# laser55/mrcAudioCodec

Measured on AMD Instinct MI355X. Metric: encode Msamples/sec (48 kHz, 2048-pt MDCT), higher is better.
Workload: dtype f64; 1 GPU; configs[1]: mono 48 kHz white noise (sigma 0.1 FS, 16-bit PCM), 2048-pt long blocks, whole encode path, independent-frames mode; hop=1024

## Files before the change

mrcaudiocodec_amd/csrc/mrc_smr_body.hpp:

```cpp
#pragma once
#include "mrc_smr_sweep.hpp"

#include <type_traits>

namespace mrc {
using namespace dev;
namespace {

constexpr int kLinesPerThread = 4;

constexpr int kSmrWavesPerSimd = 4, kSmrWavesPerSimdShort = 6;
constexpr int kFrontPrio = 3, kFarPrio = 0;

template <bool EXACT, class SampleT, int NT, int DIM, int MODE>
__device__ __forceinline__ void smr_body(DevShape S, int nsigArg, const SampleT* __restrict__ chL,
                                         const SampleT* __restrict__ chR, int64_t stride,
                                         const int64_t* __restrict__ offsetsArg, const double* __restrict__ lines,
                                         const int* __restrict__ oscale, double* __restrict__ smr,
                                         double* __restrict__ threshArg, double* __restrict__ bandPeakArg,
                                         const int* __restrict__ msSwitch, SmrLds layArg,
                                         unsigned long long* __restrict__ sens) {
    extern __shared__ double smem[];
    const SmrLds lay = DIM ? smr_layout(DIM, DIM, DIM - 100, nullptr) : layArg;
    __shared__ int waveCnt[NT / kWave];
    __shared__ unsigned long long bandKey[kMaxBands], peakKey[kMaxBands];
    __shared__ unsigned long long slopeKey[2];
    __shared__ unsigned char needBand[kMaxBands];
    const int tid = threadIdx.x;
    const int lane = tid & (kWave - 1), wave = tid >> 6;
    constexpr bool LONG = DIM == 1024;
    const int nsig = MODE == 1 ? 1 : MODE == 2 ? 4 : nsigArg;
    const bool haveSwitch = MODE == 1 ? false : MODE == 2 ? true : msSwitch != nullptr;
    const int64_t* offsets = offsetsArg;
    double* thresh = MODE ? nullptr : threshArg;
    double* bandPeak = bandPeakArg;
    const bool wantPeak = MODE ? true : bandPeakArg != nullptr;
    const int H = DIM ? DIM : S.H, M = DIM ? DIM : S.halfN;
    const int last = DIM ? DIM - 100 : S.peakLast;
    const unsigned slot = xcd_contiguous(blockIdx.x, gridDim.x);
    const int64_t f = slot / nsig;
    const int sig = (int)((slot + f) % nsig);
    const unsigned unit = (unsigned)(f * nsig + sig);
    if (haveSwitch && !thresh) {
        const bool need = lane < S.nBands && ((sig >= 2) == (msSwitch[f * S.nBands + lane] != 0));
        if (!__any(need)) return;
    }
    const int64_t off = offsets ? offsets[f] : f * stride;
    double2* A = (double2*)smem;
    double2* B = A + H;
    double* xi = smem + 4 * H;
    unsigned short* cntArr = reinterpret_cast<unsigned short*>(smem + 2 * H);
    unsigned short* nUpArr = cntArr + (M + 2);
    short* pkBin = reinterpret_cast<short*>(nUpArr + (M + 2));
    double* piHi = reinterpret_cast<double*>(pkBin + ((last / 2 + 5) & ~3));
    double* piLo = piHi + (last / 2 + 2);

#ifdef MRC_PROFILE_PHASES
    __shared__ unsigned long long sPhase_[32];
    if (threadIdx.x < 32) sPhase_[threadIdx.x] = 0ull;
    __syncthreads();
    long long tPhase_ = __builtin_readcyclecounter();
#endif
    __builtin_amdgcn_s_setprio(kFrontPrio);
    if (tid < kMaxBands) bandKey[tid] = 0ull;
    if (tid < 2) slopeKey[tid] = tid ? 0ull : ~0ull;
    if (tid < kMaxBands) peakKey[tid] = 0ull;
    if (tid < kMaxBands)
        needBand[tid] = (!haveSwitch || tid >= S.nBands) ? 1 : (((sig >= 2) == (msSwitch[f * S.nBands + tid] != 0)) ? 1 : 0);
    const double* zbS = smem + lay.zbOff;
    constexpr int TAB = (DIM == 1024 && !EXACT && NT == 256) ? kExpTabLong : kExpTab;
    constexpr int kTabLongOff = 464;
    const double* e2tab = TAB == kExpTab ? smem + 2 * H - kExpTab : smem + 4 * H + kTabLongOff;
    unsigned long long* ratioKey = reinterpret_cast<unsigned long long*>(smem + 2 * H - kExpTab - kMaxBands);
    const double* logTabLds = smem + lay.logOff;
    const double* logTab = logTabLds;
    constexpr int kPre = 4;
    const bool pairAligned = !(off & 1) && !(reinterpret_cast<uintptr_t>(chL) & (2 * sizeof(SampleT) - 1)) &&
                             (!chR || !(reinterpret_cast<uintptr_t>(chR) & (2 * sizeof(SampleT) - 1)));
    MRC_PHASE(16);
    constexpr bool kFftRegs = LONG && NT == 256 && kPre == 4;
    constexpr bool kSplitPairs = kFftRegs;
    [[maybe_unused]] double2 fftIn[4];
    [[maybe_unused]] Tw3 fftW1;
    if constexpr (kFftRegs) fftW1 = fft1024_twiddles(S.fftTw, 1, tid);
    for (int n0 = tid; n0 < H; n0 += NT * kPre) {
        double e[kPre], o[kPre], he[kPre], ho[kPre];
#pragma unroll
        for (int u = 0; u < kPre; ++u) {
            const int n = min(n0 + u * NT, H - 1);
            const double2 eo = load_signal_pair(chL, chR, off + 2 * n, sig, pairAligned);
            e[u] = eo.x;
            o[u] = eo.y;
            he[u] = S.hann[2 * n];
            ho[u] = S.hann[2 * n + 1];
        }
#pragma unroll
        for (int u = 0; u < kPre; ++u) {
            const int n = n0 + u * NT;
            if constexpr (kFftRegs) fftIn[u] = make_double2(e[u] * he[u], o[u] * ho[u]);
            else if (n < H) A[n] = make_double2(e[u] * he[u], o[u] * ho[u]);
        }
    }
    const int scale = oscale[unit];
    const double xiInv = 1.0 / S.xiDen;
    double2 wnPre[kPre];
    double zbPre[kPre], logPre = 0.0, e2Pre = 0.0;
    [[maybe_unused]] double e2Pre64 = 0.0;
#pragma unroll
    for (int u = 0; u < kPre; ++u) {
        if (!kSplitPairs || u < 2) wnPre[u] = S.wN[kSplitPairs ? tid + 1 + u * NT : min(tid + u * NT, last - 1)];
        zbPre[u] = EXACT ? 0.0 : S.zb[min(tid + u * NT, M - 1)];
    }
    if (!EXACT) {
        logPre = kLogTabDev.v[tid & (kLogTabEntries * 4 - 1)];
        e2Pre = TAB == kExpTab ? kExp2Tab[tid & (kExpTab - 1)] : kExp2Tab256[tid & 255];
        if (TAB != kExpTab) e2Pre64 = kExp2Tab[tid & (kExpTab - 1)];
    }
    double2* T;
    if constexpr (kFftRegs) {
        MRC_PHASE(0); MRC_STOP(0);
        T = fft_regs_1024(fftIn, A, B, S.fftTw, fftW1, tid);
    } else if (lay.twOff >= 0) {
        double2* Wq = reinterpret_cast<double2*>(smem + lay.twOff);
        for (int t = tid; t < H / 4; t += NT) Wq[t] = S.wH[t];
        __syncthreads();
        MRC_PHASE(0); MRC_STOP(0);
        if (LONG && NT == 256) T = fft_lds_1024<NT>(A, B, Wq, tid);
        else if (DIM == 128) T = fft_lds_128<NT>(A, B, Wq, tid);
        else
        T = fft_lds_pow2<NT>(A, B, H, S.radH, S.nRadH, TwQuarter{Wq, H / 4 - 1, 31 - __clz(H / 4)}, tid);
    } else {
        __syncthreads();
        MRC_PHASE(0); MRC_STOP(0);
        if (DIM == 576) T = fft_lds_576<NT>(A, B, S.wH, tid);
        else
        T = fft_lds_global<NT>(A, B, H, S.radH, S.nRadH, S.wH, tid);
    }
    MRC_PHASE(1); MRC_STOP(1);
    if constexpr (kSplitPairs) {
        auto intensity = [&](double2 X) {
            return EXACT ? 4. * (X.x * X.x + X.y * X.y) / S.xiDen : (4. * (X.x * X.x + X.y * X.y)) * xiInv;
        };
        auto split = [&](int k, double2 w, bool both) {
            const double2 zk = T[k];
            double2 zc = T[(H - k) & (H - 1)];
            zc.y = -zc.y;
            const double2 ev = make_double2(0.5 * (zk.x + zc.x), 0.5 * (zk.y + zc.y));
            const double2 d = make_double2(zk.x - zc.x, zk.y - zc.y);
            const double2 od = make_double2(0.5 * d.y, -0.5 * d.x);
            const double2 P = cmul(w, od);
            xi[k] = intensity(make_double2(P.x + ev.x, P.y + ev.y));
            if (both) xi[H - k] = intensity(make_double2(ev.x - P.x, ev.y - P.y));
        };
#pragma unroll
        for (int u = 0; u < 2; ++u) {
            const int k = tid + 1 + u * NT;
            split(k, wnPre[u], H - k < last && k != H / 2);
        }
        if (tid == 0) split(0, make_double2(1.0, 0.0), false);
    } else
    for (int k0 = tid; k0 < last; k0 += NT * kPre) {
        double2 wn[kPre];
#pragma unroll
        for (int u = 0; u < kPre; ++u) wn[u] = (k0 == tid) ? wnPre[u] : S.wN[min(k0 + u * NT, last - 1)];
#pragma unroll
        for (int u = 0; u < kPre; ++u) {
            const int k = k0 + u * NT;
            if (k < last) {
                double2 zk = T[k];
                double2 zc = T[(H - k) % H];
                zc.y = -zc.y;
                double2 ev = make_double2(0.5 * (zk.x + zc.x), 0.5 * (zk.y + zc.y));
                double2 d = make_double2(zk.x - zc.x, zk.y - zc.y);
                double2 od = make_double2(0.5 * d.y, -0.5 * d.x);
                double2 X = cmul(wn[u], od);
                X.x += ev.x; X.y += ev.y;
                xi[k] = EXACT ? 4. * (X.x * X.x + X.y * X.y) / S.xiDen
                              : (4. * (X.x * X.x + X.y * X.y)) * xiInv;
            }
        }
    }
    MRC_PHASE(20);
    __syncthreads();
    MRC_PHASE(2); MRC_STOP(2);
    if (!EXACT) {
        {
            double* zw = smem + lay.zbOff;
#pragma unroll
            for (int u = 0; u < kPre; ++u)
                if (tid + u * NT < M) zw[tid + u * NT] = zbPre[u];
            for (int k = tid + kPre * NT; k < M; k += NT) zw[k] = S.zb[k];
        }
        if (tid < kLogTabEntries * 4) smem[lay.logOff + tid] = logPre;
        if (tid < kExpTab) smem[2 * H - kExpTab + tid] = TAB == kExpTab ? e2Pre : e2Pre64;
        if (tid < kMaxBands) ratioKey[tid] = 0ull;
    }

    double* mt = smem;
    const int nCand = last - 2;
    const int per = (nCand + NT - 1) / NT;
    const int p0 = 1 + tid * per;
    const int p1 = min(p0 + per, last - 1);
    constexpr int kPerMax = 4;
    int mine = 0;
    unsigned flags = 0;
    if (per <= kPerMax) {
        double v[kPerMax + 2];
#pragma unroll
        for (int j = 0; j < kPerMax + 2; ++j) v[j] = xi[min(p0 - 1 + j, last - 1)];
#pragma unroll
        for (int j = 0; j < kPerMax; ++j)
            if (p0 + j < p1 && v[j + 1] > v[j] && v[j + 1] > v[j + 2]) flags |= 1u << j;
        mine = __popc(flags);
        if (sens) {
            const double kPeakGuard = 1e-11 * __longlong_as_double((long long)sens[7]);
            int near = 0;
#pragma unroll
            for (int j = 0; j < kPerMax; ++j) {
                const double c = v[j + 1], l = v[j], r = v[j + 2];
                const bool nl = fabs(c - l) <= kPeakGuard * c, nr = fabs(c - r) <= kPeakGuard * c;
                near += (p0 + j < p1 && ((nl && (c > r || nr)) || (nr && (c > l || nl)))) ? 1 : 0;
            }
            if (near) atomicAdd(&sens[3], (unsigned long long)near);
        }
    } else {
        for (int p = p0; p < p1; ++p) mine += (xi[p] > xi[p - 1] && xi[p] > xi[p + 1]) ? 1 : 0;
    }
    const int incl = wave_incl_scan(mine);
    if (lane == kWave - 1) waveCnt[wave] = incl;
    MRC_PHASE(17);
    __syncthreads();
    MRC_PHASE(18);
    int before = incl - mine, nPeaks = 0;
    for (int w = 0; w < NT / kWave; ++w) {
        const int c = waveCnt[w];
        if (w < wave) before += c;
        nPeaks += c;
    }
    if (per <= kPerMax) {
#pragma unroll
        for (int j = 0; j < kPerMax; ++j)
            if ((flags >> j) & 1u) pkBin[before++] = (short)(p0 + j);
    } else {
        for (int p = p0; p < p1; ++p)
            if (xi[p] > xi[p - 1] && xi[p] > xi[p + 1]) pkBin[before++] = (short)p;
    }
    if (!EXACT) {
        unsigned long long* z = reinterpret_cast<unsigned long long*>(cntArr);
        for (int k = tid; k < (M + 2) / 2; k += NT) z[k] = 0ull;
    }
    MRC_PHASE(19);
    __syncthreads();
    MRC_PHASE(3); MRC_STOP(3);
    double slLo = 1e300, slHi = -1e300;
    for (int mi = tid; mi < nPeaks; mi += NT) {
        const int before = mi;
        const int p = pkBin[mi];
        const double x0 = xi[p - 1], x1 = xi[p], x2 = xi[p + 1];
        {
            double s3 = (x0 + x1) + x2;
            MRC_PHASE(21);
            double level = EXACT ? spl_db(s3) : spl_db_tab(s3, logTabLds);
            const double fnum = S.binHz * (((p - 1) * x0 + p * x1) + (p + 1) * x2);
            double fm = EXACT ? fnum / s3 : fnum * recip_nr(s3);
            double q = EXACT ? fm / 7500. : fm * (1. / 7500.);
            const double zm = EXACT ? 13 * atan(0.76 * fm / 1000.) + 3.5 * atan(q * q)
                                    : 13 * atan_pos((0.76 * fm) * 1e-3) + 3.5 * atan_pos(q * q);
            const double lvl15 = level - 15.0;
            const double boost = 0.37 * fmax(level - 40, 0.0);
            double* e = mt + 4 * before;
            if (EXACT) {
                e[1] = zm;
                e[0] = lvl15;
                e[2] = boost;
            } else {
                const double xe = (lvl15 - 96) * 0.1;
                const double eh = xe * kLog2Of10;
                const double I = exp2_dd(eh, fma(xe, kLog2Of10, -eh) + xe * kLog2Of10Lo);
                const double ph = kLowHi * zm;
                const double pl = fma(kLowHi, zm, -ph) + kLowLo * zm;
                const double slope = (((-27 + boost) * 0.1) * kLog2Of10) * (double)TAB;
                slLo = fmin(slLo, slope);
                slHi = fmax(slHi, slope);
                reinterpret_cast<double2*>(e)[0] = make_double2(I, zm);
                reinterpret_cast<double2*>(e)[1] = make_double2(slope, I * exp2_dd(ph, pl));
                const int kNear = min(max((int)(fm * S.linesPerHz), 0), M - 1);
                MRC_PHASE(22);
                int lo = S.loLine[kNear], hi = S.hiLine[kNear];
#ifdef MRC_PROFILE_PHASES
                asm volatile("" : "+v"(lo), "+v"(hi));
#endif
                MRC_PHASE(23);
                {
                    auto zAt = [&](int k) { return zbS[min(max(k, 0), M - 1)]; };
                    const double a0 = zAt(lo - 2), a1 = zAt(lo - 1), a2 = zAt(lo), a3 = zAt(lo + 1);
                    const double b0 = zAt(hi - 2), b1 = zAt(hi - 1), b2 = zAt(hi), b3 = zAt(hi + 1);
                    auto sees = [&](double zv, int k) { return k >= M || (k >= 0 && zv - zm >= -0.5); };
                    auto above = [&](double zv, int k) { return k >= M || (k >= 0 && zv - zm > 0.5); };
                    const bool s0 = sees(a0, lo - 2), s1 = sees(a1, lo - 1), s2 = sees(a2, lo), s3 = sees(a3, lo + 1);
                    const bool u0 = above(b0, hi - 2), u1 = above(b1, hi - 1), u2 = above(b2, hi), u3 = above(b3, hi + 1);
                    const int first = (s1 && !s0) ? lo - 1 : (s2 && !s1) ? lo : (s3 && !s2) ? lo + 1 : -1;
                    const int over = (u1 && !u0) ? hi - 1 : (u2 && !u1) ? hi : (u3 && !u2) ? hi + 1 : -1;
                    if (__any(first < 0 || over < 0)) {
                        while (lo > 0 && zbS[lo - 1] - zm >= -0.5) --lo;
                        while (lo < M && !(zbS[lo] - zm >= -0.5)) ++lo;
                        hi = max(hi, lo);
                        while (hi > 0 && zbS[hi - 1] - zm > 0.5) --hi;
                        while (hi < M && !(zbS[hi] - zm > 0.5)) ++hi;
                    } else {
                        lo = first;
                        hi = over;
                    }
                }
                atomicAdd(reinterpret_cast<unsigned int*>(cntArr) + (lo >> 1), 1u << (16 * (lo & 1)));
                atomicAdd(reinterpret_cast<unsigned int*>(nUpArr) + (hi >> 1), 1u << (16 * (hi & 1)));
                MRC_PHASE(24);
            }
        }
    }
    if (!EXACT) {
        slLo = -wave_max(-slLo);
        slHi = wave_max(slHi);
        if (lane == 0) {
            atomicMin(&slopeKey[0], order_key(slLo));
            atomicMax(&slopeKey[1], order_key(slHi));
        }
    }
    MRC_PHASE(4);
    __syncthreads();
    MRC_PHASE(12); MRC_STOP(4);

    const double* X = lines + (int64_t)unit * M;

    if (EXACT) {
        for (int base = 0; base < M; base += NT * kLinesPerThread) {
            double z[kLinesPerThread], tot[kLinesPerThread];
#pragma unroll
            for (int j = 0; j < kLinesPerThread; ++j) {
                int k = base + tid + j * NT;
                bool ok = k < M;
                z[j] = ok ? S.zb[k] : 0.0;
                tot[j] = ok ? S.quiet[k] : 0.0;
            }
            for (int m = 0; m < nPeaks; ++m) {
                const double lvl = mt[4 * m], zm = mt[4 * m + 1], boost = mt[4 * m + 2];
#pragma unroll
                for (int j = 0; j < kLinesPerThread; ++j) {
                    double dz = z[j] - zm;
                    double adz = fabs(dz);
                    double t = adz - 0.5;
                    double arg = lvl;
                    if (adz > 0.5) arg = lvl + (-27 * t);
                    if (dz > 0.5) arg = arg + boost * t;
                    tot[j] += pow(10.0, (arg - 96) / 10);
                }
            }
#pragma unroll
            for (int j = 0; j < kLinesPerThread; ++j) {
                int k = base + tid + j * NT;
                if (k < M) {
                    double thr = spl_db(tot[j]);
                    if (thresh) thresh[(int64_t)unit * M + k] = thr;
                    double xs = ldexp(X[k], scale);
                    double spl = spl_db(2. * (xs * xs) / (1. / 2.)) - 6. * scale;
                    atomicMax(&bandKey[S.bandOfLine[k]], order_key(spl - thr));
                    if (wantPeak)
                        atomicMax(&peakKey[S.bandOfLine[k]], (unsigned long long)__double_as_longlong(fabs(X[k])));
                }
            }
        }
    } else {
        double* sc = xi;
        if (TAB != kExpTab) smem[4 * H + kTabLongOff + tid] = e2Pre;
        const int waveU = __builtin_amdgcn_readfirstlane(wave);
        const int nChunks = (M + kWave - 1) / kWave;
        const int nWaves = NT / kWave;
        struct LineConst { double z, quiet, lowE, x; int bnd; };
        auto chunk_of = [&](int i) { return i * nWaves + ((i & 1) ? (nWaves - 1 - waveU) : waveU); };
        auto load_consts = [&](int i) {
            const unsigned kc = (unsigned)min(chunk_of(i) * kWave + lane, M - 1);
            const char* lc = reinterpret_cast<const char*>(S.lineC) + kc * (unsigned)sizeof(LineConstants);
            const double2 a = *reinterpret_cast<const double2*>(lc);
            const double lowE = *reinterpret_cast<const double*>(lc + 16);
            const int bnd = *reinterpret_cast<const int*>(lc + 24);
            const double x = *reinterpret_cast<const double*>(reinterpret_cast<const char*>(X) + kc * 8u);
            return LineConst{a.x, a.y, lowE, x, bnd};
        };
        constexpr bool kFirstEarly = LONG && NT == 256;
        [[maybe_unused]] LineConst first{};
        if constexpr (kFirstEarly) first = load_consts(0);
        constexpr bool kNodes = (DIM == 1024 || DIM == 576) && NT == 256;
        constexpr int kNodeMaxMaskers = kNodes ? node_max_maskers(DIM ? DIM : 1024) : 0;
        static_assert(!kNodes || kNodeMaxMaskers >= 128, "slope nodes: too few rows for this block shape");
        [[maybe_unused]] double nodeH = 0.0, nodeS0 = 0.0;
        bool useNodes = false;
        if constexpr (kNodes) {
            const double lo = order_value(slopeKey[0]), hi = order_value(slopeKey[1]);
            nodeH = fmax((hi - lo) * (1.0 / (kNodeR - 1 - 2 * kNodeMargin)), kNodeHMin * TAB);
            nodeS0 = hi + kNodeMargin * nodeH;
            useNodes = nPeaks >= kNodeMinMaskers && nPeaks <= kNodeMaxMaskers && nodeH <= kNodeHMax * TAB;
        }
        double* const nodeQ = reinterpret_cast<double*>(pkBin);
        double* piH = piHi;
        double* piL = piLo;
        if (kNodes && useNodes) { piH = mt + 4 * nPeaks; piL = piH + (nPeaks + 1); }
        constexpr int kSegAny = DIM == 128 ? 1 : DIM == 576 ? 4 : kSmrMaxSeg;
        constexpr int kSegNodes = DIM == 1024 ? 5 : kSegAny;
        static_assert(DIM != 1024 || kWave * kSegNodes > node_max_maskers(1024), "segments of the scans");
        auto scan_sc = [&](auto segC) {
            constexpr int kSeg = decltype(segC)::value;
            double loc[kSeg];
            double run = 0.0;
            const int seg = kWave - 1 - lane;
#pragma unroll
            for (int i = kSeg - 1; i >= 0; --i) {
                const int m = seg * kSeg + i;
                run += (m < nPeaks) ? mt[4 * m + 3] : 0.0;
                loc[i] = run;
            }
            const double incl = wave_incl_scan(run);
            const double higher = dpp_shift_or_zero<0x138, 0xf>(incl);
#pragma unroll
            for (int i = 0; i < kSeg; ++i) {
                const int m = seg * kSeg + i;
                if (m < nPeaks) sc[m] = loc[i] + higher;
            }
            if (lane == 0) sc[nPeaks] = 0.0;
        };
        auto scan_pi = [&](auto segC) {
            constexpr int kSeg = decltype(segC)::value;
            double hi = 0.0, lo = 0.0, locH[kSeg], locL[kSeg];
#pragma unroll
            for (int i = 0; i < kSeg; ++i) {
                const int m = lane * kSeg + i;
                locH[i] = hi; locL[i] = lo;
                dd_add(&hi, &lo, (m < nPeaks) ? mt[4 * m] : 0.0, 0.0);
            }
            double inH = hi, inL = lo;
#define MRC_DD_SCAN_STEP(CTRL, MASK)                                                           \
            dd_add(&inH, &inL, dpp_shift_or_zero<CTRL, MASK>(inH), dpp_shift_or_zero<CTRL, MASK>(inL));
            MRC_DD_SCAN_STEP(0x111, 0xf) MRC_DD_SCAN_STEP(0x112, 0xf) MRC_DD_SCAN_STEP(0x114, 0xf)
            MRC_DD_SCAN_STEP(0x118, 0xf) MRC_DD_SCAN_STEP(0x142, 0xa) MRC_DD_SCAN_STEP(0x143, 0xc)
#undef MRC_DD_SCAN_STEP
            const double exH = dpp_shift_or_zero<0x138, 0xf>(inH), exL = dpp_shift_or_zero<0x138, 0xf>(inL);
#pragma unroll
            for (int i = 0; i < kSeg; ++i) {
                const int m = lane * kSeg + i;
                if (m <= nPeaks) {
                    double h = exH, l = exL;
                    dd_add(&h, &l, locH[i], locL[i]);
                    piH[m] = h; piL[m] = l;
                }
            }
        };
        auto scan_counts = [&](unsigned short* arr) {
            const int per2 = (M + kWave) / kWave;
            const int k0 = lane * per2, k1 = min(k0 + per2, M + 1);
            int sum = 0;
            for (int k = k0; k < k1; ++k) sum += arr[k];
            int run = wave_incl_scan(sum) - sum;
            for (int k = k0; k < k1; ++k) {
                run += arr[k];
                arr[k] = (unsigned short)run;
            }
        };
        [[maybe_unused]] auto scan_counts_1024 = [&](unsigned short* arr) {
            unsigned* w = reinterpret_cast<unsigned*>(arr) + 8 * lane;
            unsigned x[8];
#pragma unroll
            for (int j = 0; j < 8; ++j) x[j] = w[j];
            unsigned carry = 0;
#pragma unroll
            for (int j = 0; j < 8; ++j) {
                unsigned v = x[j] + (x[j] << 16);
                v += carry * 0x10001u;
                x[j] = v;
                carry = v >> 16;
            }
            const unsigned before = (unsigned)(wave_incl_scan((int)carry) - (int)carry) * 0x10001u;
#pragma unroll
            for (int j = 0; j < 8; ++j) w[j] = x[j] + before;
        };
        [[maybe_unused]] auto node_terms = [&]() {
            const double* tab64 = smem + 2 * H - kExpTab;
            const double invH = 1.0 / nodeH;
            const double s0q = nodeS0 * ((double)kExpTab / TAB), hq = nodeH * ((double)kExpTab / TAB);
            if (tid < kNodeCols) nodeQ[tid] = 0.0;
            for (int base = waveU * kWave; base < nPeaks; base += NT) {
                const int m = base + lane;
                const bool valid = m < nPeaks;
                const int mm = min(m, nPeaks - 1);
                const double2 Iz = *reinterpret_cast<const double2*>(mt + 4 * mm);
                const double I = valid ? Iz.x : 0.0, zm = Iz.y, sl = mt[4 * mm + 2];
                const double theta = (nodeS0 - sl) * invH;
                double suf[kNodeR];
                suf[kNodeR - 1] = 1.0;
#pragma unroll
                for (int r = kNodeR - 2; r >= 0; --r) suf[r] = suf[r + 1] * (theta - (r + 1));
                const double F0 = I * exp2_tab64<kExpTab>(-s0q, zm, tab64);
                const double gm = exp2_tab64<kExpTab>(hq, zm, tab64);
                double G[kNodeCols];
                double F = F0, pre = 1.0, lsum = 0.0;
#pragma unroll
                for (int r = 0; r < kNodeR; ++r) {
                    const double lam = (pre * kNodeW.c[r]) * suf[r];
                    G[r] = lam * F;
                    lsum += fabs(lam);
                    F *= gm;
                    pre *= theta - r;
                }
                G[kNodeR] = I * (fabs(pre) * kInvFactorial[kNodeR]);
                G[kNodeR + 1] = lsum * F0;
                const bool store = (lane & 3) == 0 && valid;
                double* rowOut = nodeQ + ((m >> 2) + 1) * kNodeCols;
#pragma unroll
                for (int j = 0; j < kNodeCols; ++j) {
                    double v = G[j];
                    v += dpp_move<0xB1>(v);
                    v += dpp_move<0x4E>(v);
                    if (store) rowOut[j] = v;
                }
            }
        };
        [[maybe_unused]] auto node_scan = [&](int half) {
            static_assert(kNodeCols == 18 && kNodeScanSegs * 9 <= kWave, "columns of the row scan");
            static_assert((node_max_maskers(1024) + kNodeC - 1) / kNodeC <= kNodeScanSegs * kNodeSeg, "rows of the row scan");
            const int nR = (nPeaks + kNodeC - 1) / kNodeC;
            const int L = (nR + kNodeScanSegs - 1) / kNodeScanSegs;
            const int seg = (lane * 57) >> 9;
            const int col = 9 * half + (lane - 9 * seg);
            const bool live = seg < kNodeScanSegs;
            double v[kNodeSeg];
#pragma unroll
            for (int i = 0; i < kNodeSeg; ++i) {
                const int r = 1 + seg * L + i;
                v[i] = (live && i < L && r <= nR) ? nodeQ[r * kNodeCols + col] : 0.0;
            }
#pragma unroll
            for (int i = 1; i < kNodeSeg; ++i) v[i] += v[i - 1];
            const double tot = v[kNodeSeg - 1];
            auto from_below = [&](double x, int d) {
                const int from = 4 * (lane - 9 * d);
                const double y = __hiloint2double(__builtin_amdgcn_ds_bpermute(from, __double2hiint(x)),
                                                  __builtin_amdgcn_ds_bpermute(from, __double2loint(x)));
                return seg >= d ? y : 0.0;
            };
            double off = from_below(tot, 1);
#pragma unroll
            for (int d = 1; d < kNodeScanSegs; d *= 2) off += from_below(off, d);
#pragma unroll
            for (int i = 0; i < kNodeSeg; ++i) {
                const int r = 1 + seg * L + i;
                if (live && i < L && r <= nR) nodeQ[r * kNodeCols + col] = v[i] + off;
            }
        };
        bool scansDone = false;
        if constexpr (kNodes) {
            if (useNodes) {
                MRC_PHASE(13);
                node_terms();
                MRC_PHASE(14);
                using SegN = std::integral_constant<int, kSegNodes>;
                auto counts = [&](unsigned short* arr) {
                    if constexpr (DIM == 1024) scan_counts_1024(arr); else scan_counts(arr);
                };
                if (nPeaks > NT) {
                    if (waveU == 1) scan_pi(SegN{});
                    else if (waveU == 2) { scan_sc(SegN{}); counts(cntArr); }
                    else if (waveU == 3) counts(nUpArr);
                    MRC_PHASE(9);
                    __syncthreads();
                    MRC_PHASE(15);
                    if (waveU == 2 || waveU == 3) node_scan(waveU - 2);
                } else {
                    __syncthreads();
                    MRC_PHASE(15);
                    if (waveU < 2) node_scan(waveU);
                    else if (waveU == 2) scan_pi(SegN{});
                    else { scan_sc(SegN{}); counts(cntArr); counts(nUpArr); }
                    MRC_PHASE(9);
                }
                scansDone = true;
            }
        }
        if (!scansDone) {
            for (int task = waveU; task < 4; task += NT / kWave) {
                using SegA = std::integral_constant<int, kSegAny>;
                if (task == 0) scan_sc(SegA{});
                else if (task == 1) scan_pi(SegA{});
                else if constexpr (DIM == 1024) scan_counts_1024(task == 2 ? cntArr : nUpArr);
                else scan_counts(task == 2 ? cntArr : nUpArr);
            }
        }
        __syncthreads();
        MRC_PHASE(5); MRC_STOP(5);

        auto tail_sum = [&](double tot, int cnt, int from, double lowE) {
            if (cnt > from) {
                const double ah = piH[cnt], al = piL[cnt], bh = piH[from], bl = piL[from];
                const double d1 = ah - bh;
                const double v = d1 - ah;
                const double e = ((ah - (d1 - v)) - (bh + v)) + (al - bl);
                tot += d1 + e;
            }
            return fma(lowE, sc[cnt], tot);
        };
        auto line_a2 = [&](const LineConst& cur) {
            const double xs2 = ldexp(cur.x, scale + 1);
            return xs2 * xs2;
        };
        auto line_plain = [&](double a2, double t) { return thresh != nullptr || !(a2 >= kSplFloorGuard && t >= kSplFloorGuard); };
        auto finish = [&](const LineConst& cur, int k, double t, auto noPlain) {
            const double a2 = line_a2(cur);
            const bool plain = decltype(noPlain)::value ? false : line_plain(a2, t);
            double ex = -1e300, q = 0.0;
            if (plain) {
                double thr;
                ex = excess_plain(t, a2, scale, logTab, &thr);
                if (thresh && k < M) thresh[(int64_t)unit * M + k] = thr;
            } else {
                q = line_ratio(a2, t);
            }
            const int bnd = cur.bnd;
            if (__all(bnd == __builtin_amdgcn_readfirstlane(bnd))) {
                const bool rowHead = (lane & 15) == 0;
                const double qBest = row_max(q);
                if (rowHead) atomicMax(&ratioKey[bnd], (unsigned long long)__double_as_longlong(qBest));
                if (__any(plain)) {
                    const double best = row_max(ex);
                    if (rowHead) atomicMax(&bandKey[bnd], order_key(best));
                }
                if (wantPeak) {
                    const double pk = row_max(fabs(cur.x));
                    if (rowHead) atomicMax(&peakKey[bnd], (unsigned long long)__double_as_longlong(pk));
                }
            } else {
                atomicMax(&ratioKey[bnd], (unsigned long long)__double_as_longlong(q));
                if (plain) atomicMax(&bandKey[bnd], order_key(ex));
                if (wantPeak) atomicMax(&peakKey[bnd], (unsigned long long)__double_as_longlong(fabs(cur.x)));
            }
        };
        __builtin_amdgcn_s_setprio(0);
        const double slMid = 0.5 * (order_value(slopeKey[0]) + order_value(slopeKey[1]));
        const double spreadHalf = 0.5 * (order_value(slopeKey[1]) - order_value(slopeKey[0])) * (0.6931471805599453094 / TAB);
        if (kNodes && useNodes) {
            if constexpr (kNodes) {
            MRC_NODE_COUNT(0);
            const double xr = (nodeH * kNodeR) / (-nodeS0);
            double ps = xr * xr;
            ps *= ps; ps *= ps; ps *= ps;
            const double psiStar = ps * kExpMinus16;
            struct NodeEval { double t, bound; int cnt, nUp; };
            auto node_chunk = [&](const LineConst& cur, int kc) {
                const int cnt = cntArr[kc], nUp = nUpArr[kc];
                const double zq = cur.z - 0.5;
                const int q = nUp >> 2, rem = nUp & 3;
                const double* row = nodeQ + q * kNodeCols;
                const double E0 = exp2_tab64<TAB>(nodeS0, zq, e2tab);
                const double g = exp2_tab64<TAB>(-nodeH, zq, e2tab);
                const double errBound = fma(psiStar, row[kNodeR], (kNodeRoundEps * E0) * row[kNodeR + 1]);
                const double up = node_line<kNodeC - 1, TAB>(row, mt, e2tab, 4 * q, rem, nPeaks - 1, zq, E0, g);
                return NodeEval{tail_sum(cur.quiet + up, cnt, nUp, cur.lowE), errBound, cnt, nUp};
            };
            unsigned setAside = 0;
            LineConst nxt = kFirstEarly ? first : load_consts(0);
            for (int i = 0; chunk_of(i) < nChunks; ++i) {
                const int k = chunk_of(i) * kWave + lane;
                const LineConst cur = nxt;
                nxt = load_consts(i + 1);
                if (haveSwitch && !__any(needBand[cur.bnd])) continue;
                MRC_PHASE(i == 0 ? 25 : 6);
                const NodeEval ev = node_chunk(cur, min(k, M - 1));
                MRC_PHASE(8);
                const bool odd = !(ev.bound <= kNodeTol * ev.t) || line_plain(line_a2(cur), ev.t);
                if (__any(odd)) { setAside |= 1u << i; continue; }
                MRC_NODE_COUNT(2);
                finish(cur, k, ev.t, std::true_type{});
                MRC_PHASE(10);
            }
            while (setAside) {
                const int i = __builtin_ctz(setAside);
                setAside &= setAside - 1;
                const int c = chunk_of(i);
                const int k = c * kWave + lane;
                const LineConst cur = load_consts(i);
                const NodeEval ev = node_chunk(cur, min(k, M - 1));
                double t = ev.t;
                if (__any(!(ev.bound <= kNodeTol * ev.t))) {
                    MRC_NODE_COUNT(3);
                    if (sens && lane == 0) atomicAdd(&sens[4], 1ull);
                    const double tot = cur.quiet + upper_cold<TAB>(mt, e2tab, S.zb, M, c, lane, ev.nUp, ev.cnt, cur.z, slMid, spreadHalf);
                    t = tail_sum(tot, ev.cnt, __builtin_amdgcn_readlane(ev.nUp, kWave - 1), cur.lowE);
                } else {
                    MRC_NODE_COUNT(2);
                }
                finish(cur, k, t, std::false_type{});
            }
            }
        } else {
        MRC_NODE_COUNT(1);
        for (int i0 = 0; chunk_of(i0) < nChunks; i0 += 4) {
        __builtin_amdgcn_s_setprio(kFarPrio);
        double far0 = 0.0, far1 = 0.0, far2 = 0.0, far3 = 0.0;
        unsigned farMask = 0;
        constexpr bool kHaveFar = DIM == 0 || (DIM - 101) / 2 >= kFarMinMaskers;
        for (int u = 0; kHaveFar && u < 4; ++u) {
            const int c = chunk_of(i0 + u);
            if (c >= nChunks) break;
            const int kc = min(c * kWave + lane, M - 1);
            if (haveSwitch && !__any(needBand[S.bandOfLine[kc]])) continue;
            const int nFar = __builtin_amdgcn_readfirstlane((int)nUpArr[kc]);
            double acc = 0.0;
            if (!far_eval<TAB, kHaveFar>(mt, e2tab, S.zb, M, c, lane, nFar, S.zb[kc], slMid, spreadHalf, &acc)) continue;
            farMask |= 1u << u;
            far0 = u == 0 ? acc : far0;
            far1 = u == 1 ? acc : far1;
            far2 = u == 2 ? acc : far2;
            far3 = u == 3 ? acc : far3;
        }
        MRC_PHASE(7);
        __builtin_amdgcn_s_setprio(0);
        LineConst nxt = (kFirstEarly && i0 == 0) ? first : load_consts(i0);
        for (int u = 0; u < 4; ++u) {
            const int i = i0 + u;
            const int c = chunk_of(i);
            if (c >= nChunks) break;
            const int k = c * kWave + lane;
            const int kc = min(k, M - 1);
            const LineConst cur = nxt;
            nxt = load_consts(i + 1);
            if (haveSwitch && !__any(needBand[cur.bnd])) continue;
            double tot = cur.quiet + (u == 0 ? far0 : u == 1 ? far1 : u == 2 ? far2 : far3);
            const int cnt = cntArr[kc], nUp = nUpArr[kc];
            MRC_PHASE(6);
            tot = near_eval<TAB>(mt, e2tab, nUp, cnt, cur.z - 0.5, ((farMask >> u) & 1u) != 0, tot);
            MRC_PHASE(9);
            if (MRC_PROFILE_SKIP & 8) {
                if (tot + cur.lowE + cur.x == 12345.0 && cur.bnd == 77) bandKey[0] = 1;
                continue;
            }
            finish(cur, k, tail_sum(tot, cnt, __builtin_amdgcn_readlane(nUp, kWave - 1), cur.lowE), std::false_type{});
            MRC_PHASE(10);
        }
        }
        }
    }
    __syncthreads();
    MRC_PHASE(11);
#ifdef MRC_PROFILE_PHASES
    __syncthreads();
    if (tid < 32 && (blockIdx.x & 63) == 0) atomicAdd(&gPhaseCycles[tid], tid == 31 ? 1ull : sPhase_[tid]);
#endif
    for (int bnd = tid; bnd < S.nBands; bnd += NT) {
        double v = bandKey[bnd] ? order_value(bandKey[bnd]) : -1e300;
        if (!EXACT && ratioKey[bnd]) {
            const double q = __longlong_as_double((long long)ratioKey[bnd]);
            v = fmax(v, 10 * log10_tab32(q, logTab) - 6. * scale);
        }
        smr[(int64_t)unit * S.nBands + bnd] = v;
        if (wantPeak) bandPeak[(int64_t)unit * S.nBands + bnd] = __longlong_as_double((long long)peakKey[bnd]);
    }
}

template <bool EXACT, class SampleT, int NT, int DIM, int MODE>
__global__ __launch_bounds__(NT)
__attribute__((amdgpu_waves_per_eu(DIM == 128 ? kSmrWavesPerSimdShort : kSmrWavesPerSimd,
                                   DIM == 128 ? kSmrWavesPerSimdShort : kSmrWavesPerSimd))) void smr_kernel(DevShape S, int nsigArg, const SampleT* __restrict__ chL,
                                                       const SampleT* __restrict__ chR, int64_t stride,
                                                       const int64_t* __restrict__ offsetsArg,
                                                       const double* __restrict__ lines,
                                                       const int* __restrict__ oscale, double* __restrict__ smr,
                                                       double* __restrict__ threshArg, double* __restrict__ bandPeakArg,
                                                       const int* __restrict__ msSwitch, SmrLds layArg,
                                                       unsigned long long* __restrict__ sens) {
    smr_body<EXACT, SampleT, NT, DIM, MODE>(S, nsigArg, chL, chR, stride, offsetsArg, lines, oscale, smr, threshArg,
                                            bandPeakArg, msSwitch, layArg, sens);
}

inline SmrLds smr_launch_layout(const DevShape& S, size_t* ldsBytes) {
    int total = 0;
    const SmrLds lay = smr_layout(S.H, S.halfN, S.peakLast, &total);
    *ldsBytes = (size_t)total * sizeof(double);
    return lay;
}

}
}
```

Baseline: 41400 Msamples/s.

## Prune non-contending lines with per-band lower bounds before node evaluation

In the long-block, non-exact, mode-1 path, each wave first computes a cheap lower bound on each line's signal-to-mask ratio from the quiet/tail sum and an upper bound on the masker contribution. It folds these bounds into per-band maxima in LDS. Only lines whose bound could still reach the band maximum are compacted into a list of at most one wave of contenders, and the full node evaluation runs on those alone. This is meant to cut the per-line exp/node work from four chunks per wave to about one. The cost is extra LDS atomics, fences and ballot compaction, and if there are too many contenders or the bound checks fail, everything falls back to the set-aside path.

Result: faster. 41870 Msamples/s (median of 6 runs) (+1.1%).

```diff
diff --git a/mrcaudiocodec_amd/csrc/mrc_smr_body.hpp b/mrcaudiocodec_amd/csrc/mrc_smr_body.hpp
--- a/mrcaudiocodec_amd/csrc/mrc_smr_body.hpp
+++ b/mrcaudiocodec_amd/csrc/mrc_smr_body.hpp
@@ -377,8 +377,7 @@
         const int nWaves = NT / kWave;
         struct LineConst { double z, quiet, lowE, x; int bnd; };
         auto chunk_of = [&](int i) { return i * nWaves + ((i & 1) ? (nWaves - 1 - waveU) : waveU); };
-        auto load_consts = [&](int i) {
-            const unsigned kc = (unsigned)min(chunk_of(i) * kWave + lane, M - 1);
+        auto load_line = [&](unsigned kc) {
             const char* lc = reinterpret_cast<const char*>(S.lineC) + kc * (unsigned)sizeof(LineConstants);
             const double2 a = *reinterpret_cast<const double2*>(lc);
             const double lowE = *reinterpret_cast<const double*>(lc + 16);
@@ -386,6 +385,17 @@
             const double x = *reinterpret_cast<const double*>(reinterpret_cast<const char*>(X) + kc * 8u);
             return LineConst{a.x, a.y, lowE, x, bnd};
         };
+        auto load_consts = [&](int i) { return load_line((unsigned)min(chunk_of(i) * kWave + lane, M - 1)); };
+        constexpr bool kContend = LONG && NT == 256 && !EXACT && MODE == 1;
+        constexpr int kContCap = kWave;
+        constexpr int kContLbOff = kTabLongOff + kExpTabLong, kContIdxOff = kContLbOff + (NT / kWave) * kMaxBands;
+        static_assert(!kContend || kContIdxOff + (NT / kWave) * kContCap / 4 <= DIM - 100 + 1, "contender areas: inside the spectrum");
+        [[maybe_unused]] unsigned long long* const lbKey =
+            reinterpret_cast<unsigned long long*>(smem + 4 * H + kContLbOff) + wave * kMaxBands;
+        [[maybe_unused]] unsigned short* const contIdx =
+            reinterpret_cast<unsigned short*>(smem + 4 * H + kContIdxOff) + wave * kContCap;
+        if constexpr (kContend)
+            if (lane < kMaxBands) lbKey[lane] = 0ull;
         constexpr bool kFirstEarly = LONG && NT == 256;
         [[maybe_unused]] LineConst first{};
         if constexpr (kFirstEarly) first = load_consts(0);
@@ -664,6 +674,76 @@
             };
             unsigned setAside = 0;
             LineConst nxt = kFirstEarly ? first : load_consts(0);
+            if constexpr (kContend) {
+                constexpr double kShrink = 1.0 - 0x1p-30, kFloorHi = kSplFloorGuard * (1.0 + 0x1p-30);
+                static_assert(NT / kWave == 4 && DIM / kWave == 16, "a wave's chunks: four, the i-th in lines [256 i, 256 i + 256)");
+                double a2s[4], tlb[4];
+                int bnds[4];
+#pragma unroll
+                for (int i = 0; i < 4; ++i) {
+                    const int k = chunk_of(i) * kWave + lane;
+                    const LineConst cur = nxt;
+                    if (i < 3) nxt = load_consts(i + 1);
+                    MRC_PHASE(i == 0 ? 25 : 6);
+                    const int cnt = cntArr[k], nUp = nUpArr[k];
+                    const double a2 = line_a2(cur);
+                    const double tl = tail_sum(cur.quiet, cnt, nUp, cur.lowE);
+                    const int bnd = cur.bnd;
+                    const bool oneBand = __all(bnd == __builtin_amdgcn_readfirstlane(bnd));
+                    const bool rowHead = (lane & 15) == 0;
+                    const bool whole = __any(!(a2 >= kFloorHi && tl >= kFloorHi));
+                    a2s[i] = a2; tlb[i] = tl; bnds[i] = bnd;
+                    double lb = 0.0;
+                    if (whole) setAside |= 1u << i;
+                    else {
+                        const double E0 = exp2_tab64<TAB>(nodeS0, cur.z - 0.5, e2tab);
+                        const double tub = fma(E0, nodeQ[((nUp + kNodeC - 1) >> 2) * kNodeCols + kNodeR + 1], tl);
+                        lb = (a2 * recip_nr(tub)) * kShrink;
+                    }
+                    if (oneBand) {
+                        const double pk = row_max(fabs(cur.x));
+                        if (rowHead) atomicMax(&peakKey[bnd], (unsigned long long)__double_as_longlong(pk));
+                        if (!whole) {
+                            const double best = row_max(lb);
+                            if (rowHead) atomicMax(&lbKey[bnd], (unsigned long long)__double_as_longlong(best));
+                        }
+                    } else {
+                        atomicMax(&peakKey[bnd], (unsigned long long)__double_as_longlong(fabs(cur.x)));
+                        if (!whole) atomicMax(&lbKey[bnd], (unsigned long long)__double_as_longlong(lb));
+                    }
+                    MRC_PHASE(8);
+                }
+                __builtin_amdgcn_fence(__ATOMIC_ACQ_REL, "wavefront");
+                int nCont = 0;
+#pragma unroll
+                for (int i = 0; i < 4; ++i) {
+                    if ((setAside >> i) & 1u) continue;
+                    const double L = __longlong_as_double((long long)lbKey[bnds[i]]);
+                    const bool in = !(a2s[i] < (L * tlb[i]) * kShrink);
+                    const unsigned long long m = __ballot(in);
+                    const int pos = nCont + (int)__builtin_amdgcn_mbcnt_hi((unsigned)(m >> 32), __builtin_amdgcn_mbcnt_lo((unsigned)m, 0u));
+                    if (in && pos < kContCap) contIdx[pos] = (unsigned short)(chunk_of(i) * kWave + lane);
+                    nCont += __popcll(m);
+                }
+                if (nCont > kContCap) { setAside = 0xFu; nCont = 0; }
+                __builtin_amdgcn_fence(__ATOMIC_ACQ_REL, "wavefront");
+                if (nCont > 0) {
+                    const int k = contIdx[min(lane, nCont - 1)];
+                    const LineConst cur = load_line((unsigned)k);
+                    const NodeEval ev = node_chunk(cur, k);
+                    const bool bad = !(ev.bound <= kNodeTol * ev.t);
+                    if (__any(bad)) {
+#pragma unroll
+                        for (int i = 0; i < 4; ++i)
+                            if (__any(bad && (k >> 8) == i)) setAside |= 1u << i;
+                    }
+                    MRC_NODE_COUNT(2);
+                    const bool live = !((setAside >> (k >> 8)) & 1u);
+                    const double q = live ? line_ratio(line_a2(cur), ev.t) : 0.0;
+                    atomicMax(&ratioKey[cur.bnd], (unsigned long long)__double_as_longlong(q));
+                    MRC_PHASE(10);
+                }
+            } else
             for (int i = 0; chunk_of(i) < nChunks; ++i) {
                 const int k = chunk_of(i) * kWave + lane;
                 const LineConst cur = nxt;
```
